# cloneofsimo/paint-with-words-sd

Measured on NVIDIA H100. Metric: unet_steps_per_sec_512sq_cfg, higher is better.
Workload: dtype f16

## Files before the change

paint_with_words_sd_b200/csrc/mma_sm90.cuh:

```cuda
#pragma once
#include <cuda_runtime.h>
#include <stdint.h>

#include <type_traits>

#include "pww_common.cuh"

namespace pww {
namespace ptx {

__device__ __forceinline__ uint32_t smem_u32(const void* p) { return (uint32_t)__cvta_generic_to_shared(p); }

__device__ __forceinline__ void cp_async16(uint32_t dst, const void* src, uint32_t src_bytes) {
  asm volatile("cp.async.cg.shared.global [%0], [%1], 16, %2;" ::"r"(dst), "l"(src), "r"(src_bytes) : "memory");
}
__device__ __forceinline__ void cp_async_commit() { asm volatile("cp.async.commit_group;" ::: "memory"); }
template <int N>
__device__ __forceinline__ void cp_async_wait() { asm volatile("cp.async.wait_group %0;" ::"n"(N) : "memory"); }

__device__ __forceinline__ void ldsm_x4(uint32_t addr, uint32_t& r0, uint32_t& r1, uint32_t& r2, uint32_t& r3) {
  asm volatile("ldmatrix.sync.aligned.m8n8.x4.shared.b16 {%0, %1, %2, %3}, [%4];"
               : "=r"(r0), "=r"(r1), "=r"(r2), "=r"(r3) : "r"(addr));
}
__device__ __forceinline__ void ldsm_x4_t(uint32_t addr, uint32_t& r0, uint32_t& r1, uint32_t& r2, uint32_t& r3) {
  asm volatile("ldmatrix.sync.aligned.m8n8.x4.trans.shared.b16 {%0, %1, %2, %3}, [%4];"
               : "=r"(r0), "=r"(r1), "=r"(r2), "=r"(r3) : "r"(addr));
}
__device__ __forceinline__ void ldsm_x2_t(uint32_t addr, uint32_t& r0, uint32_t& r1) {
  asm volatile("ldmatrix.sync.aligned.m8n8.x2.trans.shared.b16 {%0, %1}, [%2];" : "=r"(r0), "=r"(r1) : "r"(addr));
}

template <typename E>
__device__ __forceinline__ void mma16816(float* c, const uint32_t* a, uint32_t b0, uint32_t b1) {
  static_assert(std::is_same_v<E, __half> || std::is_same_v<E, __nv_bfloat16>, "fp16 or bf16 operands");
  if constexpr (std::is_same_v<E, __half>) {
    asm volatile(
        "mma.sync.aligned.m16n8k16.row.col.f32.f16.f16.f32 {%0, %1, %2, %3}, {%4, %5, %6, %7}, {%8, %9}, "
        "{%0, %1, %2, %3};"
        : "+f"(c[0]), "+f"(c[1]), "+f"(c[2]), "+f"(c[3])
        : "r"(a[0]), "r"(a[1]), "r"(a[2]), "r"(a[3]), "r"(b0), "r"(b1));
  } else {
    asm volatile(
        "mma.sync.aligned.m16n8k16.row.col.f32.bf16.bf16.f32 {%0, %1, %2, %3}, {%4, %5, %6, %7}, {%8, %9}, "
        "{%0, %1, %2, %3};"
        : "+f"(c[0]), "+f"(c[1]), "+f"(c[2]), "+f"(c[3])
        : "r"(a[0]), "r"(a[1]), "r"(a[2]), "r"(a[3]), "r"(b0), "r"(b1));
  }
}

__device__ __forceinline__ float ex2(float x) {
  float y;
  asm("ex2.approx.ftz.f32 %0, %1;" : "=f"(y) : "f"(x));
  return y;
}
template <typename E>
__device__ __forceinline__ uint32_t pack2(float lo, float hi) {
  const typename Elem<E>::E2 h = Elem<E>::from_float2(lo, hi);
  return *reinterpret_cast<const uint32_t*>(&h);
}
template <typename E>
__device__ __forceinline__ float2 unpack2(uint32_t v) {
  return Elem<E>::to_float2(*reinterpret_cast<const typename Elem<E>::E2*>(&v));
}
__device__ __forceinline__ unsigned long long ld_acquire_gpu_u64(const unsigned long long* p) {
  unsigned long long v;
  asm volatile("ld.acquire.gpu.global.u64 %0, [%1];" : "=l"(v) : "l"(p) : "memory");
  return v;
}

}
}
```

paint_with_words_sd_b200/csrc/pww_abi.cu:

```cuda
#include <stdio.h>
#include <string.h>

#include "pww_common.cuh"
#include "xattn_tc.cuh"
#include "xattn_fused2.cuh"
#include "attn_tc.cuh"
#include "unet_ops.cuh"
#include "sampler_step.cuh"
#include "sampler_rescale.cuh"
#include "sampler_window.cuh"
#include "control_inject.cuh"
#include "control_combine.cuh"
#include "adapter_residual.cuh"
#include <stdlib.h>
#include <algorithm>
#include <type_traits>

namespace {

thread_local char g_last_cuda_error[640] = "";

int cuda_fail(cudaError_t e);

bool aligned16(const void* p) { return (reinterpret_cast<uintptr_t>(p) & 15u) == 0; }

bool supported_head_dim(int D) { return D == 40 || D == 64 || D == 80 || D == 160; }

int check_common(const void* q, const void* k, int B, int H, int N, int T, int D, int64_t q_bs, int64_t q_rs,
                 int64_t k_bs, int64_t k_rs) {
  if (!q || !k || B <= 0 || H <= 0 || N <= 0 || T <= 0 || D <= 0) return PWW_ERR_BAD_ARG;
  if (!aligned16(q) || !aligned16(k)) return PWW_ERR_BAD_ARG;
  if ((q_bs | q_rs | k_bs | k_rs) & 7) return PWW_ERR_BAD_ARG;
  if (q_rs < (int64_t)H * D || k_rs < (int64_t)H * D) return PWW_ERR_BAD_ARG;
  if (!supported_head_dim(D) || !pww::core::supported_keys(T)) return PWW_ERR_UNSUPPORTED;
  return PWW_OK;
}

template <int D_, int KC_>
struct Shape {
  static constexpr int D = D_, KC = KC_;
};
template <int D, typename F>
cudaError_t with_chunks(int T, F&& f) {
  switch (pww::core::chunks_of(T)) {
    case 1: return f(Shape<D, 1>{});
    case 2: return f(Shape<D, 2>{});
    case 3: return f(Shape<D, 3>{});
  }
  return cudaErrorInvalidValue;
}
template <typename F>
cudaError_t with_shape(int D, int T, F&& f) {
  switch (D) {
    case 40: return with_chunks<40>(T, f);
    case 64: return with_chunks<64>(T, f);
    case 80: return with_chunks<80>(T, f);
    case 160: return with_chunks<160>(T, f);
  }
  return cudaErrorInvalidValue;
}

template <int lo, int hi, typename F>
void with_int(int v, F&& f) {
  if constexpr (lo < hi)
    if (v != lo) return with_int<lo + 1, hi>(v, f);
  f(std::integral_constant<int, lo>{});
}

size_t align_up(size_t x, size_t a) { return (x + a - 1) / a * a; }

constexpr int kStatSlotsPerImage = 2048;

int cuda_fail(cudaError_t e) {
  snprintf(g_last_cuda_error, sizeof(g_last_cuda_error), "%s: %s ", cudaGetErrorName(e), cudaGetErrorString(e));
  return PWW_ERR_CUDA;
}

template <typename E>
pww::XattnParams<E> xattn_params(const void* q, const void* k, const void* v, void* out, int B, int H, int N, int T, int D,
                                 int64_t q_bs, int64_t q_rs, int64_t k_bs, int64_t k_rs, int64_t o_bs, int64_t o_rs) {
  pww::XattnParams<E> p;
  memset(&p, 0, sizeof(p));
  p.q = (const E*)q; p.k = (const E*)k; p.v = (const E*)v; p.out = (E*)out;
  p.B = B; p.H = H; p.N = N; p.T = T; p.D = D;
  p.q_bs = q_bs; p.q_rs = q_rs; p.k_bs = k_bs; p.k_rs = k_rs; p.o_bs = o_bs; p.o_rs = o_rs;
  return p;
}

template <typename E>
pww::XattnParams<E> images(const pww::XattnParams<E>& p, int b0, int n) {
  pww::XattnParams<E> c = p;
  c.B = n;
  c.q += (int64_t)b0 * p.q_bs;
  c.k += (int64_t)b0 * p.k_bs;
  if (c.v) c.v += (int64_t)b0 * p.k_bs;
  if (c.out) c.out += (int64_t)b0 * p.o_bs;
  if (c.wmap_index) c.wmap_index += b0;
  if (c.stat_kind) c.stat_kind += b0;
  if (c.stats) c.stats += b0;
  if (c.stats_out) c.stats_out += b0;
  if (c.g_sigma) c.g_sigma += (int64_t)b0 * p.g_stride;
  return c;
}

}

extern "C" {

int pww_version(void) { return 300; }

const char* pww_status_str(int status) {
  switch (status) {
    case PWW_OK: return "ok";
    case PWW_ERR_BAD_ARG: return "bad argument (null/misaligned pointer, non-positive size or stride not a multiple of 8)";
    case PWW_ERR_UNSUPPORTED: return "unsupported shape or dtype (head dim must be 40/64/80/160, T <= 80, 154 or 231)";
    case PWW_ERR_CUDA: return "CUDA error (see pww_last_cuda_error)";
    case PWW_ERR_WORKSPACE: return "workspace too small (see pww_xattn_workspace_bytes)";
    default: return "unknown status";
  }
}

const char* pww_last_cuda_error(void) { return g_last_cuda_error; }

int pww_device_supported(void) {
  int dev = 0, major = 0;
  cudaError_t e = cudaGetDevice(&dev);
  if (e != cudaSuccess) return cuda_fail(e);
  e = cudaDeviceGetAttribute(&major, cudaDevAttrComputeCapabilityMajor, dev);
  if (e != cudaSuccess) return cuda_fail(e);
  return major == 9 ? 1 : 0;
}

size_t pww_xattn_workspace_bytes(int B, int H, int N, int T, int D) {
  (void)T; (void)D;
  if (B <= 0 || H <= 0 || N <= 0) return 0;
  return align_up((size_t)B * sizeof(unsigned int), 256) +
         (size_t)B * kStatSlotsPerImage * sizeof(pww::StatPartial);
}

}

namespace {

template <typename E>
int xattn_stats(const void* q, const void* k, int B, int H, int N, int T, int D, int64_t q_batch_stride,
                int64_t q_row_stride, int64_t k_batch_stride, int64_t k_row_stride, int stat, const int32_t* kinds,
                bool per_image, const int32_t* wmap_index, float* stats, void* workspace, size_t workspace_bytes,
                void* stream) {
  int rc = check_common(q, k, B, H, N, T, D, q_batch_stride, q_row_stride, k_batch_stride, k_row_stride);
  if (rc) return rc;
  if (!stats || !workspace) return PWW_ERR_BAD_ARG;
  if (per_image ? !kinds : (stat != PWW_STAT_MAX && stat != PWW_STAT_STD)) return PWW_ERR_BAD_ARG;
  if (workspace_bytes < pww_xattn_workspace_bytes(B, H, N, T, D)) return PWW_ERR_WORKSPACE;
  if (pww::num_sms() > kStatSlotsPerImage) return PWW_ERR_WORKSPACE;
  pww::XattnParams<E> p = xattn_params<E>(q, k, nullptr, nullptr, B, H, N, T, D, q_batch_stride, q_row_stride,
                                          k_batch_stride, k_row_stride, 0, 0);
  p.wmap_index = wmap_index; p.stat = stat; p.stat_kind = per_image ? kinds : nullptr; p.stats_out = stats;
  p.counters = (unsigned int*)workspace;
  p.partials = (pww::StatPartial*)((char*)workspace + align_up((size_t)B * sizeof(unsigned int), 256));
// ... 46 lines not shown
              rec->rec_bs < (int64_t)H * N * pww::core::kRegions))
    return PWW_ERR_BAD_ARG;
  if (mpack) {
    if (!cidx || !g_sigma || !workspace || Bw <= 0 || !aligned16(mpack)) return PWW_ERR_BAD_ARG;
    if ((mpack_batch_stride & 7) || mpack_batch_stride < (int64_t)N * pww::fx::kMW) return PWW_ERR_BAD_ARG;
    if (per_image ? !kinds : (stat != PWW_STAT_MAX && stat != PWW_STAT_STD)) return PWW_ERR_BAD_ARG;
    if (workspace_bytes < pww_xattn_fused_workspace_bytes()) return PWW_ERR_WORKSPACE;
  }
  pww::XattnParams<E> p = xattn_params<E>(q, k, v, out, B, H, N, T, D, q_batch_stride, q_row_stride, k_batch_stride,
                                          k_row_stride, o_batch_stride, o_row_stride);
  p.g_sigma = g_sigma; p.g_stride = per_image ? 1 : 0; p.scale = scale; p.stat = stat;
  p.stat_kind = per_image ? kinds : nullptr; p.stats_out = stats;
  p.wmap_index = mpack ? wmap_index : nullptr;
  p.counters = (unsigned int*)workspace;
  p.partials = workspace ? (pww::StatPartial*)((char*)workspace + 512) : nullptr;
  int chunk = pww::fx::kMaxBatch;
  const int tiles = pww::ceil_div(N, pww::core::kBM);
  const int hg = pww::ceil_div(H, D == 40 ? pww::fx::Cfg2<40>::G : (D == 64 ? pww::fx::Cfg2<64>::G : 1));
  while (chunk > 1) {
    const int cb = B < chunk ? B : chunk;
    if (pww::fx::fused2_fits(cb, hg, tiles, pww::fx::fused_grid(cb * hg * tiles))) break;
    chunk >>= 1;
  }
  for (int b0 = 0; b0 < B; b0 += chunk) {
    pww::XattnParams<E> c = images(p, b0, std::min(B - b0, chunk));
    const void* mp = mpack;
    const int8_t* ci = cidx;
    if (mpack && !wmap_index) {
      mp = (const __half*)mpack + (int64_t)b0 * mpack_batch_stride;
      ci = cidx + (int64_t)b0 * pww::core::kTP * pww::core::chunks_of(T);
    }
    c.wmap = (const float*)mp;
    pww::fx::FxRecord r;
    if (rec) {
      r = *rec;
      r.rec_index += b0;
    }
    const cudaError_t e = with_shape(D, T, [&](auto k) {
      return pww::fx::launch_fused2<k.D, k.KC>(c, mp, mpack_batch_stride, ci, (cudaStream_t)stream, rec ? &r : nullptr);
    });
    if (e == cudaErrorInvalidConfiguration) return PWW_ERR_UNSUPPORTED;
    if (e != cudaSuccess) return cuda_fail(e);
  }
  return PWW_OK;
}

template <typename E>
int groupnorm_nhwc(const void* x, const void* add, int64_t add_batch_stride, const void* gamma, const void* beta, void* y,
                   int B, int HW, int C, int G, float eps, int silu, void* workspace, size_t workspace_bytes,
                   void* stream) {
  if (!x || !gamma || !beta || !y || !workspace || B <= 0 || HW <= 0 || C <= 0 || G <= 0) return PWW_ERR_BAD_ARG;
  if (!aligned16(x) || !aligned16(y) || !aligned16(gamma) || !aligned16(beta) || (add && !aligned16(add)))
    return PWW_ERR_BAD_ARG;
  if ((C & 7) || (C % G) || G > 64 || (C >> 3) > 1024) return PWW_ERR_UNSUPPORTED;
  if (add && ((add_batch_stride & 7) || add_batch_stride < C)) return PWW_ERR_BAD_ARG;
  if (workspace_bytes < pww_groupnorm_workspace_bytes(B, HW, G)) return PWW_ERR_WORKSPACE;
  const pww::uops::GnSplit sp = pww::uops::gn_split(HW, C, G);
  pww::uops::GnParams<E> p;
  p.x = (const E*)x; p.add = (const E*)add; p.add_bs = add_batch_stride; p.gamma = (const E*)gamma; p.beta = (const E*)beta;
  p.y = (E*)y;
  p.partial = (float2*)workspace;
  p.HW = HW; p.C = C; p.G = G; p.eps = eps; p.silu = silu;
  p.sv = sp.sv; p.chunks = sp.chunks; p.rows_per_chunk = sp.rows_per_chunk;
  cudaStream_t s = (cudaStream_t)stream;
  const size_t smem1 = (64 + (size_t)2 * sp.rpp * sp.sv * 8) * sizeof(float);
  if (smem1 > 48 * 1024) {
    const cudaError_t e = pww::allow_dynamic_smem<pww::uops::gn_stats_kernel<E>>(64 * 1024 + 256);
    if (e != cudaSuccess) return cuda_fail(e);
  }
  pww::uops::gn_stats_kernel<E><<<dim3(sp.chunks, sp.slices, B), sp.threads, smem1, s>>>(p);
  int rows = 4;
  while (rows > 1 && (long long)B * sp.slices * pww::ceil_div(HW, sp.rpp * rows) < 2 * pww::num_sms()) rows >>= 1;
  cudaLaunchAttribute pdl;
  pdl.id = cudaLaunchAttributeProgrammaticStreamSerialization;
  pdl.val.programmaticStreamSerializationAllowed = 1;
  cudaLaunchConfig_t cfg = {};
  cfg.gridDim = dim3(pww::ceil_div(HW, sp.rpp * rows), sp.slices, B);
  cfg.blockDim = dim3(sp.threads);
  cfg.stream = s;
  cfg.attrs = &pdl;
  cfg.numAttrs = 1;
  cudaError_t e = cudaLaunchKernelEx(&cfg, pww::uops::gn_apply_kernel<E>, p, sp.rpp * rows);
  if (e == cudaSuccess) e = cudaGetLastError();
  return e == cudaSuccess ? PWW_OK : cuda_fail(e);
}

template <typename E>
int geglu(const void* in, void* out, int64_t M, int I, void* stream) {
  if (!in || !out || M <= 0 || I <= 0 || !aligned16(in) || !aligned16(out)) return PWW_ERR_BAD_ARG;
  if (I & 7) return PWW_ERR_UNSUPPORTED;
  const long long total = (long long)M * (I >> 3);
  long long blocks = (total + 255) / 256;
  const long long cap = (long long)pww::num_sms() * 16;
  if (blocks > cap) blocks = cap;
  pww::uops::geglu_kernel<E><<<(int)blocks, 256, 0, (cudaStream_t)stream>>>((const E*)in, (E*)out, M, I);
  cudaError_t e = cudaGetLastError();
  return e == cudaSuccess ? PWW_OK : cuda_fail(e);
}

template <typename E>
int add_layernorm(const void* x, const void* res, const void* gamma, const void* beta, void* sum_out, void* y, int64_t M,
                  int C, float eps, void* stream) {
  if (!x || !gamma || !beta || !y || M <= 0 || C <= 0) return PWW_ERR_BAD_ARG;
  if (!aligned16(x) || !aligned16(y) || !aligned16(gamma) || !aligned16(beta) || (res && !aligned16(res)) ||
      (sum_out && !aligned16(sum_out)))
    return PWW_ERR_BAD_ARG;
  if ((C & 7) || C > 2048) return PWW_ERR_UNSUPPORTED;
  const int warps = 8;
  const unsigned grid = (unsigned)((M + warps - 1) / warps);
  with_int<1, 8>(((C >> 3) + 31) / 32, [&](auto vpl) {
    pww::uops::add_layernorm_kernel<E, vpl><<<grid, warps * 32, 0, (cudaStream_t)stream>>>(
        (const E*)x, (const E*)res, (const E*)gamma, (const E*)beta, (E*)sum_out, (E*)y, M, C, eps);
  });
  cudaError_t e = cudaGetLastError();
  return e == cudaSuccess ? PWW_OK : cuda_fail(e);
}

template <typename E>
int resnet_residual(const void* a, const void* h, const float* bias, void* out, int64_t rows, int C, void* stream) {
  if (!a || !h || !bias || !out || rows <= 0 || C <= 0 || (C & 7)) return PWW_ERR_BAD_ARG;
  if (!aligned16(a) || !aligned16(h) || !aligned16(bias) || !aligned16(out)) return PWW_ERR_BAD_ARG;
  const long long total = (long long)rows * (C >> 3);
  long long blocks = (total + 255) / 256;
  const long long cap = (long long)pww::num_sms() * 16;
  if (blocks > cap) blocks = cap;
  pww::uops::resnet_residual_kernel<E><<<(int)blocks, 256, 0, (cudaStream_t)stream>>>(
      (const E*)a, (const E*)h, bias, (E*)out, total, C >> 3);
  cudaError_t e = cudaGetLastError();
  return e == cudaSuccess ? PWW_OK : cuda_fail(e);
}

template <typename E>
int adapter_residual(const void* a, const void* b, const float* bias, const void* feat, void* out, int rows,
                     int64_t pixels, int C, int feat_rows, void* stream) {
  if (!a || !b || !out || rows <= 0 || pixels <= 0 || C <= 0 || (C & 7)) return PWW_ERR_BAD_ARG;
  if (feat_rows < 0 || feat_rows > rows || (feat_rows > 0 && !feat)) return PWW_ERR_BAD_ARG;
  if (!aligned16(a) || !aligned16(b) || !aligned16(out) || (bias && !aligned16(bias)) || (feat && !aligned16(feat)))
    return PWW_ERR_BAD_ARG;
  const long long per_row = (long long)pixels * (C >> 3);
  const cudaError_t e = pww::adp::launch<E>(a, b, bias, feat, out, (long long)rows * per_row,
                                            (long long)feat_rows * per_row, C >> 3, (long long)pww::num_sms() * 16,
                                            (cudaStream_t)stream);
  return e == cudaSuccess ? PWW_OK : cuda_fail(e);
}

template <typename E>
int attn_fwd(const void* q,const void* k, const void* v, void* out, int B, int H, int N, int D, int64_t qkv_batch_stride,
             int64_t qkv_row_stride, int64_t o_batch_stride, int64_t o_row_stride, float scale, void* stream) {
  if (!q || !k || !v || !out || B <= 0 || H <= 0 || N <= 0 || D <= 0) return PWW_ERR_BAD_ARG;
  if (!aligned16(q) || !aligned16(k) || !aligned16(v) || !aligned16(out)) return PWW_ERR_BAD_ARG;
  if ((qkv_batch_stride | qkv_row_stride | o_batch_stride | o_row_stride) & 7) return PWW_ERR_BAD_ARG;
  if (qkv_row_stride < (int64_t)H * D || o_row_stride < (int64_t)H * D) return PWW_ERR_BAD_ARG;
  if (!supported_head_dim(D)) return PWW_ERR_UNSUPPORTED;
  const cudaError_t e = with_shape(D, 1, [&](auto sh) {
    return pww::fa::launch<sh.D, E>(q, k, v, out, B, H, N, qkv_batch_stride, qkv_row_stride, o_batch_stride,
                                    o_row_stride, scale, (cudaStream_t)stream);
  });
  return e == cudaSuccess ? PWW_OK : cuda_fail(e);
}

template <typename E>
int control_inject(int n, void* const* dst, const void* const* res, const int64_t* elems_per_image, int rows,
                   const float* scales, void* stream) {
  if (n < 1 || n > pww::ctl::kMaxLevels || rows < 1 || !dst || !res || !elems_per_image) return PWW_ERR_BAD_ARG;
  pww::ctl::InjectArgs a;
  a.off[0] = 0;
  for (int k = 0; k < n; ++k) {
    const int64_t e = elems_per_image[k];
    if (e <= 0 || (e % pww::ctl::kVec) != 0) return PWW_ERR_BAD_ARG;
    if (!dst[k] || !res[k] || !aligned16(dst[k]) || !aligned16(res[k])) return PWW_ERR_BAD_ARG;
    a.dst[k] = dst[k];
    a.res[k] = res[k];
    a.vec_per_image[k] = e / pww::ctl::kVec;
    a.off[k + 1] = a.off[k] + (int64_t)rows * a.vec_per_image[k];
  }
  for (int k = n; k < pww::ctl::kMaxLevels; ++k) {
    a.dst[k] = nullptr;
    a.res[k] = nullptr;
    a.vec_per_image[k] = 0;
    a.off[k + 1] = a.off[n];
  }
  a.scales = scales;
  a.n = n;
  a.rows = rows;
  const cudaError_t e = pww::ctl::launch_inject<E>(a, (int64_t)pww::num_sms() * 8, (cudaStream_t)stream);
  return e == cudaSuccess ? PWW_OK : cuda_fail(e);
}

template <typename E>
int control_combine(int units, int n, void* const* out, const void* const* res, const int64_t* elems_per_image,
                    int rows, const float* scales, void* stream) {
  if (units < 1 || units > pww::ctl::kMaxUnits || n < 1 || n > pww::ctl::kMaxLevels || rows < 1 || !out || !res ||
      !elems_per_image || !scales)
    return PWW_ERR_BAD_ARG;
  pww::ctl::CombineArgs a = {};
  for (int k = 0; k < n; ++k) {
    const int64_t e = elems_per_image[k];
    if (e <= 0 || (e % pww::ctl::kVec) != 0) return PWW_ERR_BAD_ARG;
    if (!out[k] || !aligned16(out[k])) return PWW_ERR_BAD_ARG;
    a.out[k] = out[k];
    a.vec_per_image[k] = e / pww::ctl::kVec;
    a.off[k + 1] = a.off[k] + (int64_t)rows * a.vec_per_image[k];
  }
  for (int i = 0; i < units * n; ++i) {
    if (!res[i] || !aligned16(res[i])) return PWW_ERR_BAD_ARG;
    a.res[i] = res[i];
  }
  for (int k = n; k < pww::ctl::kMaxLevels; ++k) a.off[k + 1] = a.off[n];
  a.scales = scales;
  a.units = units;
  a.n = n;
  a.rows = rows;
  const cudaError_t e = pww::ctl::launch_combine<E>(a, (int64_t)pww::num_sms() * 8, (cudaStream_t)stream);
  return e == cudaSuccess ? PWW_OK : cuda_fail(e);
}

}

extern "C" {

int pww_xattn_stats_f16(const void* q, const void* k, int B, int H, int N, int T, int D, int64_t q_batch_stride,
    int64_t q_row_stride, int64_t k_batch_stride, int64_t k_row_stride, int stat, const int32_t* wmap_index,
    float* stats, void* workspace, size_t workspace_bytes, void* stream) {
  return xattn_stats<__half>(
      q, k, B, H, N, T, D, q_batch_stride, q_row_stride, k_batch_stride, k_row_stride, stat, nullptr, false,
      wmap_index, stats, workspace, workspace_bytes, stream);
}
int pww_xattn_stats_bf16(const void* q, const void* k, int B, int H, int N, int T, int D, int64_t q_batch_stride,
    int64_t q_row_stride, int64_t k_batch_stride, int64_t k_row_stride, int stat, const int32_t* wmap_index,
    float* stats, void* workspace, size_t workspace_bytes, void* stream) {
  return xattn_stats<__nv_bfloat16>(
      q, k, B, H, N, T, D, q_batch_stride, q_row_stride, k_batch_stride, k_row_stride, stat, nullptr, false,
      wmap_index, stats, workspace, workspace_bytes, stream);
}

int pww_xattn_stats_multi_f16(const void* q, const void* k, int B, int H, int N, int T, int D, int64_t q_batch_stride,
    int64_t q_row_stride, int64_t k_batch_stride, int64_t k_row_stride, const int32_t* stat, const int32_t* wmap_index,
    float* stats, void* workspace, size_t workspace_bytes, void* stream) {
  return xattn_stats<__half>(
      q, k, B, H, N, T, D, q_batch_stride, q_row_stride, k_batch_stride, k_row_stride, PWW_STAT_MAX, stat, true,
      wmap_index, stats, workspace, workspace_bytes, stream);
}
int pww_xattn_stats_multi_bf16(const void* q, const void* k, int B, int H, int N, int T, int D, int64_t q_batch_stride,
    int64_t q_row_stride, int64_t k_batch_stride, int64_t k_row_stride, const int32_t* stat, const int32_t* wmap_index,
    float* stats, void* workspace, size_t workspace_bytes, void* stream) {
  return xattn_stats<__nv_bfloat16>(
      q, k, B, H, N, T, D, q_batch_stride, q_row_stride, k_batch_stride, k_row_stride, PWW_STAT_MAX, stat, true,
      wmap_index, stats, workspace, workspace_bytes, stream);
}

int pww_xattn_fwd_f16(const void* q, const void* k, const void* v, void* out, int B, int H, int N, int T, int D,
    int64_t q_batch_stride, int64_t q_row_stride, int64_t k_batch_stride, int64_t k_row_stride, int64_t o_batch_stride,
    int64_t o_row_stride, const float* wmap, int64_t wmap_batch_stride, const int32_t* wmap_index, const float* stats,
    const float* g_sigma, float scale, void* stream) {
  return xattn_fwd<__half>(q, k, v, out, B, H, N, T, D, q_batch_stride, q_row_stride, k_batch_stride, k_row_stride,
      o_batch_stride, o_row_stride, wmap, wmap_batch_stride, wmap_index, stats, g_sigma, 0, scale, stream);
}
int pww_xattn_fwd_bf16(const void* q, const void* k, const void* v, void* out, int B, int H, int N, int T, int D,
    int64_t q_batch_stride, int64_t q_row_stride, int64_t k_batch_stride, int64_t k_row_stride, int64_t o_batch_stride,
    int64_t o_row_stride, const float* wmap, int64_t wmap_batch_stride, const int32_t* wmap_index, const float* stats,
    const float* g_sigma, float scale, void* stream) {
  return xattn_fwd<__nv_bfloat16>(
      q, k, v, out, B, H, N, T, D, q_batch_stride, q_row_stride, k_batch_stride, k_row_stride,
      o_batch_stride, o_row_stride, wmap, wmap_batch_stride, wmap_index, stats, g_sigma, 0, scale, stream);
}

int pww_xattn_fwd_multi_f16(const void* q, const void* k, const void* v, void* out, int B, int H, int N, int T, int D,
    int64_t q_batch_stride, int64_t q_row_stride, int64_t k_batch_stride, int64_t k_row_stride, int64_t o_batch_stride,
    int64_t o_row_stride, const float* wmap, int64_t wmap_batch_stride, const int32_t* wmap_index, const float* stats,
    const float* g_sigma, float scale, void* stream) {
  return xattn_fwd<__half>(q, k, v, out, B, H, N, T, D, q_batch_stride, q_row_stride, k_batch_stride, k_row_stride,
      o_batch_stride, o_row_stride, wmap, wmap_batch_stride, wmap_index, stats, g_sigma, 1, scale, stream);
}
int pww_xattn_fwd_multi_bf16(const void* q, const void* k, const void* v, void* out, int B, int H, int N, int T, int D,
    int64_t q_batch_stride, int64_t q_row_stride, int64_t k_batch_stride, int64_t k_row_stride, int64_t o_batch_stride,
    int64_t o_row_stride, const float* wmap, int64_t wmap_batch_stride, const int32_t* wmap_index, const float* stats,
    const float* g_sigma, float scale, void* stream) {
  return xattn_fwd<__nv_bfloat16>(
      q, k, v, out, B, H, N, T, D, q_batch_stride, q_row_stride, k_batch_stride, k_row_stride,
      o_batch_stride, o_row_stride, wmap, wmap_batch_stride, wmap_index, stats, g_sigma, 1, scale, stream);
}

size_t pww_xattn_fused_workspace_bytes(void) { return pww::fx::fused_workspace_bytes(); }

int pww_xattn_fused_f16(const void* q, const void* k, const void* v, void* out, int B, int H, int N, int T, int D,
    int64_t q_batch_stride, int64_t q_row_stride, int64_t k_batch_stride, int64_t k_row_stride, int64_t o_batch_stride,
    int64_t o_row_stride, const void* mpack, int64_t mpack_batch_stride, int Bw, const int8_t* cidx,
    const int32_t* wmap_index, int stat, const float* g_sigma, float scale, float* stats, void* workspace,
    size_t workspace_bytes, void* stream) {
  return xattn_fused<__half>(q, k, v, out, B, H, N, T, D, q_batch_stride, q_row_stride, k_batch_stride, k_row_stride,
      o_batch_stride, o_row_stride, mpack, mpack_batch_stride, Bw, cidx, wmap_index, stat, nullptr, false,
      g_sigma, scale, stats, workspace, workspace_bytes, stream);
}
int pww_xattn_fused_bf16(const void* q, const void* k, const void* v, void* out, int B, int H, int N, int T, int D,
    int64_t q_batch_stride, int64_t q_row_stride, int64_t k_batch_stride, int64_t k_row_stride, int64_t o_batch_stride,
    int64_t o_row_stride, const void* mpack, int64_t mpack_batch_stride, int Bw, const int8_t* cidx,
    const int32_t* wmap_index, int stat, const float* g_sigma, float scale, float* stats, void* workspace,
    size_t workspace_bytes, void* stream) {
  return xattn_fused<__nv_bfloat16>(
      q, k, v, out, B, H, N, T, D, q_batch_stride, q_row_stride, k_batch_stride, k_row_stride,
      o_batch_stride, o_row_stride, mpack, mpack_batch_stride, Bw, cidx, wmap_index, stat, nullptr, false,
      g_sigma, scale, stats, workspace, workspace_bytes, stream);
}

int pww_xattn_fused_multi_f16(const void* q, const void* k, const void* v, void* out, int B, int H, int N, int T, int D,
    int64_t q_batch_stride, int64_t q_row_stride, int64_t k_batch_stride, int64_t k_row_stride, int64_t o_batch_stride,
    int64_t o_row_stride, const void* mpack, int64_t mpack_batch_stride, int Bw, const int8_t* cidx,
    const int32_t* wmap_index, const int32_t* stat, const float* g_sigma, float scale, float* stats, void* workspace,
    size_t workspace_bytes, void* stream) {
  return xattn_fused<__half>(q, k, v, out, B, H, N, T, D, q_batch_stride, q_row_stride, k_batch_stride, k_row_stride,
// ... 318 lines not shown
```

paint_with_words_sd_b200/csrc/xattn_core.cuh:

```cuda
#pragma once
#include "mma_sm90.cuh"
#include "pww_common.cuh"

namespace pww {
namespace core {

constexpr int kBM = 128;
constexpr int kTP = 80;
constexpr int kWarps = 8;
constexpr int kThreads = kWarps * 32;

template <int D>
struct Tile {
  static_assert(D == 40 || D == 64 || D == 80 || D == 160, "head dims of SD1.5 (40 / 80 / 160) and SD2.x (64)");
  static constexpr int DP = (D + 15) / 16 * 16;
  static constexpr int LD = DP + 8;
  static constexpr int KS = DP / 16;
  static constexpr int NT = D / 8;
  static constexpr uint32_t QBYTES = kBM * LD * 2;
  static constexpr uint32_t KBYTES = kTP * LD * 2;
};

template <int D, typename E>
__device__ __forceinline__ void load_rows(uint32_t dst, const E* src, int64_t rs, int nrows, int valid) {
  using C = Tile<D>;
  constexpr int CH = C::DP / 8, DCH = D / 8;
  for (int idx = threadIdx.x; idx < nrows * CH; idx += blockDim.x) {
    const int r = idx / CH, c = idx - r * CH;
    const bool ok = r < valid && c < DCH;
    ptx::cp_async16(dst + (uint32_t)(r * C::LD + c * 8) * 2u, ok ? (const void*)(src + (int64_t)r * rs + c * 8) : (const void*)src,
                    ok ? 16u : 0u);
  }
}

template <int D, typename E>
__device__ __forceinline__ void warp_qk(uint32_t qs, uint32_t ks, int lane, float (&s)[10][4]) {
  using C = Tile<D>;
#pragma unroll
  for (int j = 0; j < 10; ++j) s[j][0] = s[j][1] = s[j][2] = s[j][3] = 0.f;
#pragma unroll
  for (int kk = 0; kk < C::KS; ++kk) {
    uint32_t a[4];
    ptx::ldsm_x4(qs + (uint32_t)((lane & 15) * C::LD + kk * 16 + (lane >> 4) * 8) * 2u, a[0], a[1], a[2], a[3]);
#pragma unroll
    for (int jp = 0; jp < 5; ++jp) {
      const int t = 16 * jp + (lane & 7) + ((lane >> 4) << 3), d = kk * 16 + ((lane >> 3) & 1) * 8;
      uint32_t b0, b1, b2, b3;
      ptx::ldsm_x4(ks + (uint32_t)(t * C::LD + d) * 2u, b0, b1, b2, b3);
      ptx::mma16816<E>(s[2 * jp], a, b0, b1);
      ptx::mma16816<E>(s[2 * jp + 1], a, b2, b3);
    }
  }
}

__device__ __forceinline__ int tok(int j, int e, int lane) { return 8 * j + 2 * (lane & 3) + (e & 1); }

template <int D, typename E>
__device__ __forceinline__ void warp_store(const float (&o)[Tile<D>::NT][4], unsigned char* stage, int lane, E* out,
                                           int64_t o_rs, int row0, int N) {
  using C = Tile<D>;
  __syncwarp();
  const int g = lane >> 2, q = lane & 3;
#pragma unroll
  for (int j = 0; j < C::NT; ++j) {
    *reinterpret_cast<uint32_t*>(stage + (g * C::LD + 8 * j + 2 * q) * 2) = ptx::pack2<E>(o[j][0], o[j][1]);
    *reinterpret_cast<uint32_t*>(stage + ((g + 8) * C::LD + 8 * j + 2 * q) * 2) = ptx::pack2<E>(o[j][2], o[j][3]);
  }
  __syncwarp();
  for (int idx = lane; idx < 16 * C::NT; idx += 32) {
    const int r = idx / C::NT, c = idx - r * C::NT;
    if (row0 + r < N)
      *reinterpret_cast<uint4*>(out + (int64_t)(row0 + r) * o_rs + c * 8) =
          *reinterpret_cast<const uint4*>(stage + (r * C::LD + c * 8) * 2);
  }
  __syncwarp();
}

constexpr int kChunk = 77;
constexpr int kMaxChunks = 3;
__host__ __device__ __forceinline__ constexpr int chunks_of(int T) { return T <= kTP ? 1 : T / kChunk; }
__host__ __device__ __forceinline__ constexpr bool supported_keys(int T) {
  return T <= kTP || T == 2 * kChunk || T == kMaxChunks * kChunk;
}
template <int KC>
__host__ __device__ __forceinline__ constexpr int chunk_keys(int T) { return KC == 1 ? T : kChunk; }

template <int D, int KC, typename E>
__device__ __forceinline__ void load_operands(uint32_t st, const XattnParams<E>& p, int b, int h, int tile, bool with_v) {
  using C = Tile<D>;
  const int rows = p.N - tile * kBM;
  load_rows<D>(st, p.q + (int64_t)b * p.q_bs + (int64_t)tile * kBM * p.q_rs + h * D, p.q_rs, kBM, rows < kBM ? rows : kBM);
  const int kv = chunk_keys<KC>(p.T);
#pragma unroll 1
  for (int c = 0; c < KC; ++c) {
    const int64_t off = (int64_t)b * p.k_bs + (int64_t)c * kChunk * p.k_rs + h * D;
    load_rows<D>(st + C::QBYTES + c * C::KBYTES, p.k + off, p.k_rs, kTP, kv);
    if (with_v) load_rows<D>(st + C::QBYTES + (KC + c) * C::KBYTES, p.v + off, p.k_rs, kTP, kv);
  }
}

template <int D>
__device__ __forceinline__ void warp_online_begin(float (&o)[Tile<D>::NT][4], float& m0, float& m1, float& l0, float& l1) {
#pragma unroll
  for (int j = 0; j < Tile<D>::NT; ++j) o[j][0] = o[j][1] = o[j][2] = o[j][3] = 0.f;
  m0 = m1 = -INFINITY;
  l0 = l1 = 0.f;
}

struct NoPHook {
  template <int NK>
  __device__ __forceinline__ void operator()(const uint32_t (&)[NK][4], float, float) const {}
};

template <int D, typename E, int NJ, typename Hook = NoPHook>
__device__ __forceinline__ void warp_online_chunk(float (&s)[NJ][4], int kv, float sl2, uint32_t vs, int lane,
                                                  float (&o)[Tile<D>::NT][4], float& m0, float& m1, float& l0, float& l1,
                                                  const Hook& hook = Hook{}) {
  static_assert(NJ % 2 == 0, "P V takes two n-tiles of P per k-step");
  using C = Tile<D>;
  float t0 = -INFINITY, t1 = -INFINITY;
#pragma unroll
  for (int j = 0; j < NJ; ++j)
#pragma unroll
    for (int e = 0; e < 4; ++e) {
      if (tok(j, e, lane) >= kv) s[j][e] = -INFINITY;
      if (e < 2) t0 = fmaxf(t0, s[j][e]); else t1 = fmaxf(t1, s[j][e]);
    }
  t0 = fmaxf(t0, __shfl_xor_sync(0xffffffffu, t0, 1));
  t0 = fmaxf(t0, __shfl_xor_sync(0xffffffffu, t0, 2));
  t1 = fmaxf(t1, __shfl_xor_sync(0xffffffffu, t1, 1));
  t1 = fmaxf(t1, __shfl_xor_sync(0xffffffffu, t1, 2));
  const float mn0 = fmaxf(m0, t0), mn1 = fmaxf(m1, t1);
  const float a0 = ptx::ex2((m0 - mn0) * sl2), a1 = ptx::ex2((m1 - mn1) * sl2);
  m0 = mn0; m1 = mn1;
  const float n0 = -mn0 * sl2, n1 = -mn1 * sl2;
  uint32_t pa[NJ / 2][4];
  float r0 = 0.f, r1 = 0.f;
#pragma unroll
  for (int j = 0; j < NJ; ++j) {
    const uint32_t p01 = ptx::pack2<E>(ptx::ex2(fmaf(s[j][0], sl2, n0)), ptx::ex2(fmaf(s[j][1], sl2, n0)));
    const uint32_t p23 = ptx::pack2<E>(ptx::ex2(fmaf(s[j][2], sl2, n1)), ptx::ex2(fmaf(s[j][3], sl2, n1)));
    const float2 f01 = ptx::unpack2<E>(p01), f23 = ptx::unpack2<E>(p23);
    r0 += f01.x + f01.y;
    r1 += f23.x + f23.y;
    pa[j >> 1][(j & 1) * 2] = p01;
    pa[j >> 1][(j & 1) * 2 + 1] = p23;
  }
  l0 = l0 * a0 + r0;
  l1 = l1 * a1 + r1;
#pragma unroll
  for (int j = 0; j < C::NT; ++j) {
    o[j][0] *= a0; o[j][1] *= a0; o[j][2] *= a1; o[j][3] *= a1;
  }
#pragma unroll
  for (int kk = 0; kk < NJ / 2; ++kk) {
    const int t = 16 * kk + (lane & 7) + ((lane >> 3) & 1) * 8;
#pragma unroll
    for (int jp = 0; jp < C::NT / 2; ++jp) {
      uint32_t b0, b1, b2, b3;
      ptx::ldsm_x4_t(vs + (uint32_t)(t * C::LD + 16 * jp + (lane >> 4) * 8) * 2u, b0, b1, b2, b3);
      ptx::mma16816<E>(o[2 * jp], pa[kk], b0, b1);
      ptx::mma16816<E>(o[2 * jp + 1], pa[kk], b2, b3);
    }
    if constexpr (C::NT & 1) {
      uint32_t b0, b1;
      ptx::ldsm_x2_t(vs + (uint32_t)(t * C::LD + 8 * (C::NT - 1)) * 2u, b0, b1);
      ptx::mma16816<E>(o[C::NT - 1], pa[kk], b0, b1);
    }
  }
  hook(pa, a0, a1);
}

template <int D>
__device__ __forceinline__ void warp_online_end(float (&o)[Tile<D>::NT][4], float l0, float l1) {
  l0 += __shfl_xor_sync(0xffffffffu, l0, 1);
  l0 += __shfl_xor_sync(0xffffffffu, l0, 2);
  l1 += __shfl_xor_sync(0xffffffffu, l1, 1);
  l1 += __shfl_xor_sync(0xffffffffu, l1, 2);
  const float i0 = 1.f / l0, i1 = 1.f / l1;
#pragma unroll
  for (int j = 0; j < Tile<D>::NT; ++j) {
    o[j][0] *= i0; o[j][1] *= i0; o[j][2] *= i1; o[j][3] *= i1;
  }
}

constexpr int kRegions = 16;

template <typename E, int NK>
__device__ __forceinline__ void warp_region_chunk(const uint32_t (&pa)[NK][4], float a0, float a1, const int8_t* rt,
                                                  int lane, float (&rm)[2][4]) {
#pragma unroll
  for (int j = 0; j < 2; ++j) {
    rm[j][0] *= a0; rm[j][1] *= a0; rm[j][2] *= a1; rm[j][3] *= a1;
  }
  const int r = lane >> 2;
#pragma unroll
  for (int kk = 0; kk < NK; ++kk) {
    const int t = 16 * kk + 2 * (lane & 3);
    const int i0 = __ldg(rt + t), i1 = __ldg(rt + t + 1), i2 = __ldg(rt + t + 8), i3 = __ldg(rt + t + 9);
#pragma unroll
    for (int j = 0; j < 2; ++j) {
      const int slot = r + 8 * j;
      const uint32_t b0 = ptx::pack2<E>(i0 == slot ? 1.f : 0.f, i1 == slot ? 1.f : 0.f);
      const uint32_t b1 = ptx::pack2<E>(i2 == slot ? 1.f : 0.f, i3 == slot ? 1.f : 0.f);
      ptx::mma16816<E>(rm[j], pa[kk], b0, b1);
    }
  }
}

__device__ __forceinline__ void warp_region_add(const float (&rm)[2][4], float l0, float l1, float* acc, int row0, int N,
                                                int lane) {
  l0 += __shfl_xor_sync(0xffffffffu, l0, 1);
  l0 += __shfl_xor_sync(0xffffffffu, l0, 2);
  l1 += __shfl_xor_sync(0xffffffffu, l1, 1);
  l1 += __shfl_xor_sync(0xffffffffu, l1, 2);
  const float inv[2] = {1.f / l0, 1.f / l1};
  const int g = lane >> 2, q = lane & 3;
#pragma unroll
  for (int hf = 0; hf < 2; ++hf) {
    const int row = row0 + g + 8 * hf;
    if (row >= N) continue;
    float* a = acc + (int64_t)row * kRegions + 2 * q;
#pragma unroll
    for (int j = 0; j < 2; ++j) {
      a[8 * j] += rm[j][2 * hf] * inv[hf];
      a[8 * j + 1] += rm[j][2 * hf + 1] * inv[hf];
    }
  }
}

template <typename E>
__device__ __forceinline__ void warp_stat(const float (&s)[10][4], int T, int rows_left, int lane, bool is_max, float& vmax,
                                          float& sum, float& sumsq) {
  const int g = lane >> 2;
#pragma unroll
  for (int j = 0; j < 10; ++j)
#pragma unroll
    for (int e = 0; e < 4; ++e) {
      const bool ok = tok(j, e, lane) < T && (g + (e >> 1) * 8) < rows_left;
      if (is_max) {
        if (ok) vmax = fmaxf(vmax, s[j][e]);
      } else if (ok) {
        const float h = round_to<E>(s[j][e]);
        sum += h;
        sumsq = fmaf(h, h, sumsq);
      }
    }
}

__device__ __forceinline__ void warp_reduce_stat(double& m, double& a, double& q) {
#pragma unroll
  for (int o = 16; o > 0; o >>= 1) {
    m = fmax(m, __shfl_xor_sync(0xffffffffu, m, o));
    a += __shfl_xor_sync(0xffffffffu, a, o);
    q += __shfl_xor_sync(0xffffffffu, q, o);
  }
}

template <typename E>
__device__ __forceinline__ float stat_value(const XattnParams<E>& p, bool is_max, double m, double a, double q) {
  const double cnt = (double)p.H * (double)p.N * (double)p.T;
  double r;
  if (is_max) {
    r = m;
  } else {
    const double var = (q - a * a / cnt) / (cnt - 1.0);
    r = sqrt(var > 0.0 ? var : 0.0);
  }
  return round_to<E>((float)r);
}

}
}
```

Measured before the change: 160.5.

## Add warp-specialized wgmma self-attention kernel for head dim 40

Adds a Hopper wgmma-based flash attention kernel for D=40. A dedicated producer warp loads K/V tiles into a multi-stage shared-memory ring, signalled through named barriers, while two consumer warpgroups run asynchronous wgmma for QK^T and PV with register-resident P. The online softmax is factored out of the shared core so it can be reused, and gains an unmasked variant for full key tiles. The aim is higher tensor-core throughput than mma.sync for the largest-resolution self-attention layers. The trade-offs are added barrier and sync complexity and serialized wgmma waits with no overlap inside a warpgroup.

```diff
diff --git a/paint_with_words_sd_b200/csrc/attn_wgmma.cuh b/paint_with_words_sd_b200/csrc/attn_wgmma.cuh
--- /dev/null
+++ b/paint_with_words_sd_b200/csrc/attn_wgmma.cuh
@@ -0,0 +1,191 @@
+#pragma once
+#include "mma_sm90.cuh"
+#include "pww_common.cuh"
+#include "xattn_core.cuh"
+
+namespace pww {
+namespace wg {
+
+constexpr int D = 40;
+constexpr int kWarpgroups = 2;
+constexpr int kConsumerWarps = kWarpgroups * 4;
+constexpr int kThreads = kConsumerWarps * 32 + 32;
+constexpr int kBM = kWarpgroups * 64;
+constexpr int kBN = 64;
+constexpr int kRound = 3;
+constexpr int kStages = 2 * kRound;
+static_assert(kBM == core::kBM, "the Q tile is the shared block's");
+using QT = core::Tile<D>;
+
+template <int COLS>
+struct KeyTile {
+  static constexpr uint32_t kPlane = kBN * 16;
+  static constexpr uint32_t kBytes = COLS / 8 * kPlane;
+  static constexpr __host__ __device__ uint32_t offset(int t, int c) { return (uint32_t)c * kPlane + (uint32_t)t * 16u; }
+};
+using KTile = KeyTile<QT::DP>;
+using VTile = KeyTile<D>;
+constexpr uint32_t kCoreBytes = 128, kCoreRows = 8;
+static_assert(KTile::offset(kCoreRows, 0) == kCoreBytes && VTile::offset(kCoreRows, 0) == kCoreBytes,
+              "8 keys of a plane are one 128-byte core matrix");
+static_assert(KTile::offset(0, 1) == KTile::kPlane && KTile::kPlane % kCoreBytes == 0, "planes of whole core matrices");
+static_assert(KTile::kPlane < (1u << 18), "descriptor offsets are 14 bits of 16-byte units");
+constexpr uint32_t kKLbo = KTile::kPlane, kKSbo = kCoreBytes;
+constexpr uint32_t kVLbo = kCoreBytes, kVSbo = VTile::kPlane;
+constexpr uint32_t kKStep = 2 * KTile::kPlane;
+constexpr uint32_t kVStep = 2 * kCoreBytes;
+static_assert(QT::KS == 3 && QT::DP == 48, "3 k-steps over d padded to 48");
+
+struct Cfg {
+  static constexpr uint32_t STAGE = KTile::kBytes + VTile::kBytes;
+  static constexpr uint32_t OFF_KV = QT::QBYTES;
+  static constexpr uint32_t SMEM = QT::QBYTES + kStages * STAGE;
+  static_assert(OFF_KV % 128 == 0 && STAGE % 128 == 0, "core matrices on 128-byte boundaries");
+  static_assert(2 * SMEM <= 232448 - 2 * 1024, "two CTAs per SM");
+};
+
+template <typename E>
+struct Params {
+  const E* q;
+  const E* k;
+  const E* v;
+  E* out;
+  int B, H, N;
+  int64_t bs, rs;
+  int64_t o_bs, o_rs;
+  float scale;
+};
+
+__device__ __forceinline__ int full_bar(int s) { return 1 + s; }
+__device__ __forceinline__ int empty_bar(int s) { return 1 + kStages + s; }
+static_assert(1 + 2 * kStages <= 16, "16 named barriers per CTA");
+__device__ __forceinline__ void bar_sync(int id) { asm volatile("bar.sync %0, %1;" ::"r"(id), "n"(kThreads) : "memory"); }
+__device__ __forceinline__ void bar_arrive(int id) { asm volatile("bar.arrive %0, %1;" ::"r"(id), "n"(kThreads) : "memory"); }
+
+template <typename E>
+__global__ void __launch_bounds__(kThreads, 2) attn_wgmma_kernel(const Params<E> p) {
+  extern __shared__ __align__(128) unsigned char smem[];
+  const uint32_t smem0 = ptx::smem_u32(smem);
+  const int warp = threadIdx.x >> 5, lane = threadIdx.x & 31;
+  const int qtiles = (p.N + kBM - 1) / kBM;
+  const int bh = blockIdx.x / qtiles, qt = blockIdx.x - bh * qtiles;
+  const int b = bh / p.H, h = bh - b * p.H;
+  const int row_base = qt * kBM;
+  const E* qb = p.q + (int64_t)b * p.bs + h * D;
+  const int ntiles = (p.N + kBN - 1) / kBN;
+  for (int i = threadIdx.x; i < kStages * (int)(KTile::kPlane / 16); i += kThreads) {
+    const int st = i / (KTile::kPlane / 16), r = i - st * (KTile::kPlane / 16);
+    *reinterpret_cast<uint4*>(smem + Cfg::OFF_KV + st * Cfg::STAGE + (QT::DP / 8 - 1) * KTile::kPlane + r * 16) =
+        make_uint4(0u, 0u, 0u, 0u);
+  }
+  {
+    const int rows = p.N - row_base < kBM ? p.N - row_base : kBM;
+    core::load_rows<D>(smem0, qb + (int64_t)row_base * p.rs, p.rs, kBM, rows);
+    ptx::cp_async_commit();
+    ptx::cp_async_wait<0>();
+    ptx::fence_proxy_async();
+    __syncthreads();
+  }
+
+  if (warp == kConsumerWarps) {
+    const E* kb = p.k + (int64_t)b * p.bs + h * D;
+    const E* vb = p.v + (int64_t)b * p.bs + h * D;
+#pragma unroll 1
+    for (int r0 = 0; r0 < ntiles; r0 += kRound) {
+      const int r1 = r0 + kRound < ntiles ? r0 + kRound : ntiles;
+#pragma unroll 1
+      for (int j = r0; j < r1; ++j) {
+        if (j >= kStages) bar_sync(empty_bar(j % kStages));
+        const uint32_t ks = smem0 + Cfg::OFF_KV + (uint32_t)(j % kStages) * Cfg::STAGE, vs = ks + KTile::kBytes;
+        const int rows = p.N - j * kBN < kBN ? p.N - j * kBN : kBN;
+        const E* kt = kb + (int64_t)j * kBN * p.rs;
+        const E* vt = vb + (int64_t)j * kBN * p.rs;
+        constexpr int CH = D / 8;
+        for (int idx = lane; idx < kBN * CH; idx += 32) {
+          const int t = idx / CH, c = idx - t * CH;
+          const bool ok = t < rows;
+          const int64_t src = ok ? (int64_t)t * p.rs + c * 8 : 0;
+          ptx::cp_async16(ks + KTile::offset(t, c), kt + src, ok ? 16u : 0u);
+          ptx::cp_async16(vs + VTile::offset(t, c), vt + src, ok ? 16u : 0u);
+        }
+      }
+      ptx::cp_async_commit();
+      ptx::cp_async_wait<0>();
+      ptx::fence_proxy_async();
+#pragma unroll 1
+      for (int j = r0; j < r1; ++j) bar_arrive(full_bar(j % kStages));
+    }
+    return;
+  }
+
+  uint32_t qa[QT::KS][4];
+  {
+    const uint32_t qs = smem0 + (uint32_t)(warp * 16 * QT::LD) * 2u;
+#pragma unroll
+    for (int kk = 0; kk < QT::KS; ++kk)
+      ptx::ldsm_x4(qs + (uint32_t)((lane & 15) * QT::LD + kk * 16 + (lane >> 4) * 8) * 2u, qa[kk][0], qa[kk][1],
+                   qa[kk][2], qa[kk][3]);
+  }
+  float o[QT::NT][4], m0, m1, l0, l1;
+  core::warp_online_begin<D>(o, m0, m1, l0, l1);
+  float s[kBN / 8][4];
+#pragma unroll
+  for (int j = 0; j < kBN / 8; ++j) s[j][0] = s[j][1] = s[j][2] = s[j][3] = 0.f;
+  const float sl2 = p.scale * 1.4426950408889634f;
+#pragma unroll 1
+  for (int jt = 0; jt < ntiles; ++jt) {
+    const int st = jt % kStages;
+    bar_sync(full_bar(st));
+    const uint32_t ks = smem0 + Cfg::OFF_KV + (uint32_t)st * Cfg::STAGE, vs = ks + KTile::kBytes;
+    ptx::wgmma_fence();
+    ptx::wgmma_m64n64k16<E, 0, 0>(s, qa[0], ptx::smem_desc(ks, kKLbo, kKSbo));
+    ptx::wgmma_m64n64k16<E, 1, 0>(s, qa[1], ptx::smem_desc(ks + kKStep, kKLbo, kKSbo));
+    ptx::wgmma_m64n64k16<E, 1, 0>(s, qa[2], ptx::smem_desc(ks + 2 * kKStep, kKLbo, kKSbo));
+    ptx::wgmma_commit();
+    ptx::wgmma_wait<0>();
+#pragma unroll
+    for (int j = 0; j < kBN / 8; ++j)
+#pragma unroll
+      for (int e = 0; e < 4; ++e) ptx::reg_fence(s[j][e]);
+    const int kv = p.N - jt * kBN;
+    uint32_t pa[kBN / 16][4];
+    float a0, a1;
+    if (kv < kBN) core::online_softmax<D, E>(s, kv, sl2, lane, o, m0, m1, l0, l1, pa, a0, a1);
+    else core::online_softmax<D, E, kBN / 8, false>(s, kv, sl2, lane, o, m0, m1, l0, l1, pa, a0, a1);
+    ptx::wgmma_fence();
+#pragma unroll
+    for (int kk = 0; kk < kBN / 16; ++kk)
+      ptx::wgmma_m64n40k16<E, 1, 1>(o, pa[kk], ptx::smem_desc(vs + kk * kVStep, kVLbo, kVSbo));
+    ptx::wgmma_commit();
+    ptx::wgmma_wait<0>();
+#pragma unroll
+    for (int kk = 0; kk < kBN / 16; ++kk)
+#pragma unroll
+      for (int e = 0; e < 4; ++e) ptx::reg_fence(pa[kk][e]);
+#pragma unroll
+    for (int j = 0; j < QT::NT; ++j)
+#pragma unroll
+      for (int e = 0; e < 4; ++e) ptx::reg_fence(o[j][e]);
+    if (jt + kStages < ntiles) bar_arrive(empty_bar(st));
+  }
+  core::warp_online_end<D>(o, l0, l1);
+  core::warp_store<D>(o, smem + warp * 16 * QT::LD * 2, lane, p.out + (int64_t)b * p.o_bs + h * D, p.o_rs,
+                      row_base + warp * 16, p.N);
+}
+
+template <typename E>
+cudaError_t launch(const void* q, const void* k, const void* v, void* out, int B, int H, int N, int64_t bs, int64_t rs,
+                   int64_t o_bs, int64_t o_rs, float scale, cudaStream_t s) {
+  Params<E> p;
+  p.q = (const E*)q; p.k = (const E*)k; p.v = (const E*)v; p.out = (E*)out;
+  p.B = B; p.H = H; p.N = N; p.bs = bs; p.rs = rs; p.o_bs = o_bs; p.o_rs = o_rs; p.scale = scale;
+  const cudaError_t e = allow_dynamic_smem<attn_wgmma_kernel<E>>(Cfg::SMEM);
+  if (e != cudaSuccess) return e;
+  const long long grid = (long long)B * H * ((N + kBM - 1) / kBM);
+  if (grid > 0x7fffffffLL) return cudaErrorInvalidConfiguration;
+  attn_wgmma_kernel<E><<<(unsigned)grid, kThreads, Cfg::SMEM, s>>>(p);
+  return cudaGetLastError();
+}
+
+}
+}
diff --git a/paint_with_words_sd_b200/csrc/mma_sm90.cuh b/paint_with_words_sd_b200/csrc/mma_sm90.cuh
--- a/paint_with_words_sd_b200/csrc/mma_sm90.cuh
+++ b/paint_with_words_sd_b200/csrc/mma_sm90.cuh
@@ -48,6 +48,54 @@
   }
 }
 
+__device__ __forceinline__ void wgmma_fence() { asm volatile("wgmma.fence.sync.aligned;" ::: "memory"); }
+__device__ __forceinline__ void wgmma_commit() { asm volatile("wgmma.commit_group.sync.aligned;" ::: "memory"); }
+template <int N>
+__device__ __forceinline__ void wgmma_wait() { asm volatile("wgmma.wait_group.sync.aligned %0;" ::"n"(N) : "memory"); }
+__device__ __forceinline__ void reg_fence(float& r) { asm volatile("" : "+f"(r)::"memory"); }
+__device__ __forceinline__ void reg_fence(uint32_t& r) { asm volatile("" : "+r"(r)::"memory"); }
+__device__ __forceinline__ void fence_proxy_async() { asm volatile("fence.proxy.async.shared::cta;" ::: "memory"); }
+
+__device__ __forceinline__ uint64_t smem_desc(uint32_t addr, uint32_t lbo, uint32_t sbo) {
+  return (uint64_t)((addr & 0x3FFFFu) >> 4) | ((uint64_t)(lbo >> 4) << 16) | ((uint64_t)(sbo >> 4) << 32);
+}
+
+template <typename E, int ACC, int TB>
+__device__ __forceinline__ void wgmma_m64n64k16(float (&d)[8][4], const uint32_t (&a)[4], uint64_t b) {
+  static_assert(std::is_same_v<E, __half> || std::is_same_v<E, __nv_bfloat16>, "fp16 or bf16 operands");
+#define PWW_WGMMA_N64(T)                                                                                              \
+  asm volatile(                                                                                                       \
+      "{\n.reg .pred p;\nsetp.ne.b32 p, %38, 0;\n"                                                                    \
+      "wgmma.mma_async.sync.aligned.m64n64k16.f32." T "." T " "                                                       \
+      "{%0, %1, %2, %3, %4, %5, %6, %7, %8, %9, %10, %11, %12, %13, %14, %15, "                                       \
+      "%16, %17, %18, %19, %20, %21, %22, %23, %24, %25, %26, %27, %28, %29, %30, %31}, "                             \
+      "{%32, %33, %34, %35}, %36, p, 1, 1, %37;\n}\n"                                                                  \
+      : "+f"(d[0][0]), "+f"(d[0][1]), "+f"(d[0][2]), "+f"(d[0][3]), "+f"(d[1][0]), "+f"(d[1][1]), "+f"(d[1][2]),     \
+        "+f"(d[1][3]), "+f"(d[2][0]), "+f"(d[2][1]), "+f"(d[2][2]), "+f"(d[2][3]), "+f"(d[3][0]), "+f"(d[3][1]),     \
+        "+f"(d[3][2]), "+f"(d[3][3]), "+f"(d[4][0]), "+f"(d[4][1]), "+f"(d[4][2]), "+f"(d[4][3]), "+f"(d[5][0]),     \
+        "+f"(d[5][1]), "+f"(d[5][2]), "+f"(d[5][3]), "+f"(d[6][0]), "+f"(d[6][1]), "+f"(d[6][2]), "+f"(d[6][3]),     \
+        "+f"(d[7][0]), "+f"(d[7][1]), "+f"(d[7][2]), "+f"(d[7][3])                                                    \
+      : "r"(a[0]), "r"(a[1]), "r"(a[2]), "r"(a[3]), "l"(b), "n"(TB), "r"(ACC))
+  if constexpr (std::is_same_v<E, __half>) PWW_WGMMA_N64("f16"); else PWW_WGMMA_N64("bf16");
+#undef PWW_WGMMA_N64
+}
+template <typename E, int ACC, int TB>
+__device__ __forceinline__ void wgmma_m64n40k16(float (&d)[5][4], const uint32_t (&a)[4], uint64_t b) {
+  static_assert(std::is_same_v<E, __half> || std::is_same_v<E, __nv_bfloat16>, "fp16 or bf16 operands");
+#define PWW_WGMMA_N40(T)                                                                                              \
+  asm volatile(                                                                                                       \
+      "{\n.reg .pred p;\nsetp.ne.b32 p, %26, 0;\n"                                                                    \
+      "wgmma.mma_async.sync.aligned.m64n40k16.f32." T "." T " "                                                       \
+      "{%0, %1, %2, %3, %4, %5, %6, %7, %8, %9, %10, %11, %12, %13, %14, %15, %16, %17, %18, %19}, "                  \
+      "{%20, %21, %22, %23}, %24, p, 1, 1, %25;\n}\n"                                                                  \
+      : "+f"(d[0][0]), "+f"(d[0][1]), "+f"(d[0][2]), "+f"(d[0][3]), "+f"(d[1][0]), "+f"(d[1][1]), "+f"(d[1][2]),     \
+        "+f"(d[1][3]), "+f"(d[2][0]), "+f"(d[2][1]), "+f"(d[2][2]), "+f"(d[2][3]), "+f"(d[3][0]), "+f"(d[3][1]),     \
+        "+f"(d[3][2]), "+f"(d[3][3]), "+f"(d[4][0]), "+f"(d[4][1]), "+f"(d[4][2]), "+f"(d[4][3])                     \
+      : "r"(a[0]), "r"(a[1]), "r"(a[2]), "r"(a[3]), "l"(b), "n"(TB), "r"(ACC))
+  if constexpr (std::is_same_v<E, __half>) PWW_WGMMA_N40("f16"); else PWW_WGMMA_N40("bf16");
+#undef PWW_WGMMA_N40
+}
+
 __device__ __forceinline__ float ex2(float x) {
   float y;
   asm("ex2.approx.ftz.f32 %0, %1;" : "=f"(y) : "f"(x));
diff --git a/paint_with_words_sd_b200/csrc/pww_abi.cu b/paint_with_words_sd_b200/csrc/pww_abi.cu
--- a/paint_with_words_sd_b200/csrc/pww_abi.cu
+++ b/paint_with_words_sd_b200/csrc/pww_abi.cu
@@ -5,6 +5,7 @@
 #include "xattn_tc.cuh"
 #include "xattn_fused2.cuh"
 #include "attn_tc.cuh"
+#include "attn_wgmma.cuh"
 #include "unet_ops.cuh"
 #include "sampler_step.cuh"
 #include "sampler_rescale.cuh"
@@ -357,10 +358,15 @@
   if ((qkv_batch_stride | qkv_row_stride | o_batch_stride | o_row_stride) & 7) return PWW_ERR_BAD_ARG;
   if (qkv_row_stride < (int64_t)H * D || o_row_stride < (int64_t)H * D) return PWW_ERR_BAD_ARG;
   if (!supported_head_dim(D)) return PWW_ERR_UNSUPPORTED;
-  const cudaError_t e = with_shape(D, 1, [&](auto sh) {
-    return pww::fa::launch<sh.D, E>(q, k, v, out, B, H, N, qkv_batch_stride, qkv_row_stride, o_batch_stride,
-                                    o_row_stride, scale, (cudaStream_t)stream);
-  });
+  const cudaError_t e =
+      D == pww::wg::D
+          ? pww::wg::launch<E>(q, k, v, out, B, H, N, qkv_batch_stride, qkv_row_stride, o_batch_stride, o_row_stride,
+                               scale, (cudaStream_t)stream)
+          : with_shape(D, 1, [&](auto sh) {
+              if constexpr (decltype(sh)::D == pww::wg::D) return cudaErrorInvalidValue;
+              else return pww::fa::launch<decltype(sh)::D, E>(q, k, v, out, B, H, N, qkv_batch_stride, qkv_row_stride,
+                                                             o_batch_stride, o_row_stride, scale, (cudaStream_t)stream);
+            });
   return e == cudaSuccess ? PWW_OK : cuda_fail(e);
 }
 
diff --git a/paint_with_words_sd_b200/csrc/xattn_core.cuh b/paint_with_words_sd_b200/csrc/xattn_core.cuh
--- a/paint_with_words_sd_b200/csrc/xattn_core.cuh
+++ b/paint_with_words_sd_b200/csrc/xattn_core.cuh
@@ -112,18 +112,17 @@
   __device__ __forceinline__ void operator()(const uint32_t (&)[NK][4], float, float) const {}
 };
 
-template <int D, typename E, int NJ, typename Hook = NoPHook>
-__device__ __forceinline__ void warp_online_chunk(float (&s)[NJ][4], int kv, float sl2, uint32_t vs, int lane,
-                                                  float (&o)[Tile<D>::NT][4], float& m0, float& m1, float& l0, float& l1,
-                                                  const Hook& hook = Hook{}) {
+template <int D, typename E, int NJ, bool MASK = true>
+__device__ __forceinline__ void online_softmax(float (&s)[NJ][4], int kv, float sl2, int lane,
+                                               float (&o)[Tile<D>::NT][4], float& m0, float& m1, float& l0, float& l1,
+                                               uint32_t (&pa)[NJ / 2][4], float& a0, float& a1) {
   static_assert(NJ % 2 == 0, "P V takes two n-tiles of P per k-step");
-  using C = Tile<D>;
   float t0 = -INFINITY, t1 = -INFINITY;
 #pragma unroll
   for (int j = 0; j < NJ; ++j)
 #pragma unroll
     for (int e = 0; e < 4; ++e) {
-      if (tok(j, e, lane) >= kv) s[j][e] = -INFINITY;
+      if (MASK && tok(j, e, lane) >= kv) s[j][e] = -INFINITY;
       if (e < 2) t0 = fmaxf(t0, s[j][e]); else t1 = fmaxf(t1, s[j][e]);
     }
   t0 = fmaxf(t0, __shfl_xor_sync(0xffffffffu, t0, 1));
@@ -131,10 +130,10 @@
   t1 = fmaxf(t1, __shfl_xor_sync(0xffffffffu, t1, 1));
   t1 = fmaxf(t1, __shfl_xor_sync(0xffffffffu, t1, 2));
   const float mn0 = fmaxf(m0, t0), mn1 = fmaxf(m1, t1);
-  const float a0 = ptx::ex2((m0 - mn0) * sl2), a1 = ptx::ex2((m1 - mn1) * sl2);
+  a0 = ptx::ex2((m0 - mn0) * sl2);
+  a1 = ptx::ex2((m1 - mn1) * sl2);
   m0 = mn0; m1 = mn1;
   const float n0 = -mn0 * sl2, n1 = -mn1 * sl2;
-  uint32_t pa[NJ / 2][4];
   float r0 = 0.f, r1 = 0.f;
 #pragma unroll
   for (int j = 0; j < NJ; ++j) {
@@ -149,9 +148,19 @@
   l0 = l0 * a0 + r0;
   l1 = l1 * a1 + r1;
 #pragma unroll
-  for (int j = 0; j < C::NT; ++j) {
+  for (int j = 0; j < Tile<D>::NT; ++j) {
     o[j][0] *= a0; o[j][1] *= a0; o[j][2] *= a1; o[j][3] *= a1;
   }
+}
+
+template <int D, typename E, int NJ, typename Hook = NoPHook>
+__device__ __forceinline__ void warp_online_chunk(float (&s)[NJ][4], int kv, float sl2, uint32_t vs, int lane,
+                                                  float (&o)[Tile<D>::NT][4], float& m0, float& m1, float& l0, float& l1,
+                                                  const Hook& hook = Hook{}) {
+  using C = Tile<D>;
+  uint32_t pa[NJ / 2][4];
+  float a0, a1;
+  online_softmax<D, E>(s, kv, sl2, lane, o, m0, m1, l0, l1, pa, a0, a1);
 #pragma unroll
   for (int kk = 0; kk < NJ / 2; ++kk) {
     const int t = 16 * kk + (lane & 7) + ((lane >> 3) & 1) * 8;
```

Result: no change. 160.8, median of 6 (+0.2%).
